# Accenture/AmpliGraph

Measured on AMD Instinct MI355X. Metric: training triples/sec (incl. negatives), ComplEx k=200 eta=20 FB15K-237-shaped, higher is better.
Workload: dtype f32; 1 GPU; synth-fb15k237 (uniform, seed 0) ComplEx k=200 eta=20 self_adversarial adam lr=1e-3, 10000 positives/GPU/step, tables resident in HBM, dense (non-lazy) Keras-legacy Adam every step; preset=C2, optimizer_mode=dense, deterministic=False, global_batch=10000, n_ents=14505, n_rels=237, row_floats=400, stored_row_floats=400, parallelism=single GPU

## Files before the change

### ampligraph_amd/csrc/kge_train_common.h

```cpp
#pragma once

#define KGE_FAST_ROTATE 1

#include "kge_device.h"
#include "kge_host.h"
#include "kge_loss.h"

static_assert(kge::ROTATE_FAST_FORMS, "kge_device.h was included before kge_train_common.h: this unit would train RotatE with the exact sqrt / division forms");

namespace kge {

struct __attribute__((aligned(16))) StageEntry {
    uint32_t pos;
    uint32_t meta;
    float g;
    uint32_t dest;
};

constexpr uint32_t ENTRY_LOCAL_MASK = 0x1FFFu;
__host__ __device__ __forceinline__ uint32_t entry_local(uint32_t meta) { return (meta >> 2) & ENTRY_LOCAL_MASK; }
constexpr int ENTRY_J_SHIFT = 16;

constexpr int LOSS_PARTS = 64;
constexpr int LOSS_PART_STRIDE = 16;

#ifndef KGE_TILE_RB
#define KGE_TILE_RB 8
#endif
constexpr uint32_t TILE_RB = KGE_TILE_RB;
__host__ __device__ __forceinline__ void tile_of_row(uint32_t row, uint32_t n_tiles, uint32_t rb, uint32_t& tile, uint32_t& local) {
    const uint32_t blk = row / rb;
    tile = blk % n_tiles;
    local = (blk / n_tiles) * rb + row % rb;
}
__host__ __device__ __forceinline__ int64_t row_of_tile(uint32_t tile, uint32_t local, uint32_t n_tiles, uint32_t rb) {
    return ((int64_t)(local / rb) * n_tiles + tile) * rb + local % rb;
}

constexpr int HOT_MAX = 64;
constexpr int HOT_REPL = 16;

struct TrainArgs {
    const float* ent;
    const float* rel;
    const float* rel_cs;
    const int32_t* triples;
    const int32_t* neg_override;
    float* g_ent;
    float* g_rel;
    double* loss_sum;
    double* loss_parts;
    float* pos_scores;
    float* neg_scores;
    int64_t B;
    int eta;
    int k;
    int K;
    int k_live;
    int nq;
    SampleCfg sc;
    ModelConst mc;
    amdkge_loss loss;
    float* stage_rows;
    int pos_atomic;
    int sign_off;
    int ns;
    int det;
    const uint8_t* hot_map;
    float* hot_buf;
    uint8_t* touched;
    uint32_t* sign_codes;
    StageEntry* st_lists;
    StageEntry* st_ovf;
    int* st_counters;
    int st_tile_rows, st_n_tiles, st_cap, st_ovf_cap, st_rb;
#ifdef KGE_ABLATE
    int dbg;
#endif
};

#ifdef KGE_ABLATE
#define KGE_DBG(a, bit) (((a).dbg & (bit)) != 0)
#else
#define KGE_DBG(a, bit) false
#endif

__device__ __forceinline__ void fold_loss_parts(double* parts, double* loss_sum, int lane, int lane_in_slot = 0) {
    static_assert(LOSS_PARTS == KGE_WAVE, "one partial per lane");
    const unsigned long long old = atomicExch(reinterpret_cast<unsigned long long*>(parts + (size_t)lane * LOSS_PART_STRIDE + lane_in_slot), 0ull);
    double t = __longlong_as_double((long long)old);
#pragma unroll
    for (int o = 32; o > 0; o >>= 1) t += __shfl_xor(t, o, 64);
    if (lane == 0 && loss_sum && t != 0.0) atomicAdd(loss_sum, t);
}

struct WaveWalk {
    float* sn;
    int lane;
    __device__ __forceinline__ int first() const { return lane; }
    __device__ __forceinline__ int stride() const { return KGE_WAVE; }
    __device__ __forceinline__ float load(int j) const { return sn[j]; }
    __device__ __forceinline__ void store(int j, float v) const { sn[j] = v; }
    __device__ __forceinline__ float sum(float v) const { return wave_sum(v); }
    __device__ __forceinline__ float max(float v) const { return wave_max(v); }
};

__device__ __forceinline__ bool entry_wanted(float coeff, float g) {
    return !(fabsf(g) < 1.17549435e-38f) || __float_as_uint(coeff) == 0x80000000u;
}


__device__ __forceinline__ void stage_draws(const TrainArgs& a, int64_t i, int ps, int first, int stride, int* sh_keep, int* sh_repl) {
    for (int j = first; j < a.eta; j += stride) {
        int keep, repl;
        if (a.neg_override) {
            const int64_t r = (int64_t)j * a.B + i;
            const int ns = a.neg_override[3 * r + 0], no = a.neg_override[3 * r + 2];
            keep = (ns == ps) ? 1 : 0;
            repl = keep ? no : ns;
        } else {
            draw_corruption(a.sc, i, j, keep, repl);
        }
        sh_keep[j] = keep;
        sh_repl[j] = repl;
    }
}

template <int MODEL>
__device__ __forceinline__ void stage_side_rows(const float (&s)[4][ModelTraits<MODEL>::NC], const float (&p)[4][ModelTraits<MODEL>::NC],
                                                const float (&o)[4][ModelTraits<MODEL>::NC], float* qa, float* qb, int k) {
    constexpr int NC = ModelTraits<MODEL>::NC;
    float va[NC][4], vb[NC][4];
#pragma unroll
    for (int u = 0; u < 4; ++u) {
        if constexpr (MODEL == AMDKGE_DISTMULT || MODEL == AMDKGE_COMPLEX) {
            float ds[NC], dp[NC], dd[NC];
            grad_unit<MODEL>(s[u], p[u], o[u], 1.f, ds, dp, dd);
#pragma unroll
            for (int h = 0; h < NC; ++h) { va[h][u] = dd[h]; vb[h][u] = ds[h]; }
        } else if constexpr (MODEL == AMDKGE_ROTATE) {
            const float cs = p[u][0], sn = p[u][1];
            va[0][u] = s[u][0] * cs - s[u][1] * sn; va[1][u] = s[u][0] * sn + s[u][1] * cs;
            vb[0][u] = o[u][0] * cs + o[u][1] * sn; vb[1][u] = o[u][1] * cs - o[u][0] * sn;
        } else {
#pragma unroll
            for (int h = 0; h < NC; ++h) { va[h][u] = s[u][h]; vb[h][u] = o[u][h]; }
        }
    }
#pragma unroll
    for (int h = 0; h < NC; ++h) {
        *reinterpret_cast<float4*>(qa + h * k) = make_float4(va[h][0], va[h][1], va[h][2], va[h][3]);
        *reinterpret_cast<float4*>(qb + h * k) = make_float4(vb[h][0], vb[h][1], vb[h][2], vb[h][3]);
    }
}

__device__ __forceinline__ void stage_append(const TrainArgs& a, int64_t i, uint32_t role, float g, uint32_t dest) {
    uint32_t tile, local;
    tile_of_row(dest, (uint32_t)a.st_n_tiles, (uint32_t)a.st_rb, tile, local);
    StageEntry* where;
    const int slotpos = atomicAdd(a.st_counters + (size_t)tile * 32, 1);
    if (slotpos < a.st_cap) {
        where = a.st_lists + (size_t)tile * a.st_cap + slotpos;
    } else {
        const int op = atomicAdd(a.st_counters + (size_t)a.st_n_tiles * 32, 1);
        if (op >= a.st_ovf_cap) return;
        where = a.st_ovf + op;
    }
    *where = StageEntry{(uint32_t)i, role | (local << 2), g, dest};
}

__host__ __device__ inline size_t sign_stash_bytes(int model, int eta, int CH) {
    return model == AMDKGE_TRANSE ? (size_t)256 * eta * CH : 0;
}

__host__ __device__ inline size_t slot_lds_bytes(int eta, int W) {
    const size_t b = (size_t)(eta + 1) * (3 + (W > 1 ? W : 2) + 1) * 4 + 8 + (W > 1 ? 64 * 4 : 0);
    return (b + 7) & ~(size_t)7;
}

template <int W>
__device__ __forceinline__ void slot_sync() {
    if constexpr (W == 1) {
        __builtin_amdgcn_fence(__ATOMIC_ACQ_REL, "wavefront");
        __builtin_amdgcn_wave_barrier();
    } else {
        __syncthreads();
    }
}

}
```

### ampligraph_amd/csrc/kge_train_kernel.h

```cpp
#pragma once
#include "kge_train_common.h"

namespace kge {

__device__ __forceinline__ void focus_apply(int nl, float x, float wgt, float& y, float& dfac) {
    float f, fp;
    switch (nl) {
        case AMDKGE_FOCUS_TANH: f = tanhf(x); fp = 1.f - f * f; break;
        case AMDKGE_FOCUS_SIGMOID: f = sigmoidf(x); fp = f * (1.f - f); break;
        case AMDKGE_FOCUS_SOFTPLUS: { const float e = 9999.f * expf(x); f = logf(1.f + e); fp = 1.f - 1.f / (1.f + e); } break;
        default: f = x; fp = 1.f; break;
    }
    y = f * wgt;
    dfac = fp * wgt;
}

struct OnePassState {
    float m;
    float S, Lw, Zs;
};

__device__ __forceinline__ float fast_exp(float x) {
    const float t = x * 1.4426950216293335f;
    const float r = fmaf(x, 1.4426950216293335f, -t) + x * 1.9259629911266175e-8f;
    const float v = __builtin_amdgcn_exp2f(t) * fmaf(r, 0.6931471805599453f, 1.f);
    return (x < -110.f) ? 0.f : v;
}
__device__ __forceinline__ void fast_sig_logsig(float y, float& sig, float& logsig_neg) {
    const float t = fast_exp(-fabsf(y));
    const float u = 1.f + t;
    const float r = __builtin_amdgcn_rcpf(u);
    sig = (y >= 0.f) ? r : t * r;
    logsig_neg = fminf(-y, 0.f) - (__builtin_amdgcn_logf(u) * 0.6931471805599453f + (t - (u - 1.f)) * r);
}

__device__ __forceinline__ float det_exp(float x) {
    x = (x != x) ? x : fminf(fmaxf(x, -80.f), 80.f);
    const float n = rintf(x * 1.4426950216293335f);
    const float r = (x - n * 0.693359375f) - n * -2.12194440e-4f;
    float p = 1.f / 5040.f;
    p = p * r + 1.f / 720.f;
    p = p * r + 1.f / 120.f;
    p = p * r + 1.f / 24.f;
    p = p * r + 1.f / 6.f;
    p = p * r + 0.5f;
    p = p * r + 1.f;
    p = p * r + 1.f;
    return ldexpf(p, (int)n);
}
__device__ __forceinline__ float det_log12(float u) {
    const float z = (u - 1.f) / (u + 1.f);
    const float w = z * z;
    float p = 1.f / 15.f;
    p = p * w + 1.f / 13.f;
    p = p * w + 1.f / 11.f;
    p = p * w + 1.f / 9.f;
    p = p * w + 1.f / 7.f;
    p = p * w + 1.f / 5.f;
    p = p * w + 1.f / 3.f;
    p = p * w + 1.f;
    return (2.f * z) * p;
}
__device__ __forceinline__ void det_sig_logsig(float y, float& sig, float& logsig_neg) {
    const float t = det_exp(-fabsf(y));
    const float u = 1.f + t;
    sig = (y >= 0.f) ? 1.f / u : t / u;
    logsig_neg = fminf(-y, 0.f) - (det_log12(u) + (t - (u - 1.f)) / u);
}
__device__ __forceinline__ void sig_logsig(bool det, float y, float& sig, float& logsig_neg) {
    if (det) det_sig_logsig(y, sig, logsig_neg); else fast_sig_logsig(y, sig, logsig_neg);
}
__device__ __forceinline__ float exp_any(bool det, float x) { return det ? det_exp(x) : fast_exp(x); }

__device__ __forceinline__ float onepass_coeff(const amdkge_loss& L, float P, float n, bool valid, OnePassState& st,
                                               float& c1, float& c2, bool det = false) {
    c1 = 0.f;
    c2 = 0.f;
    float rescale = 1.f;
    switch (L.kind) {
        case AMDKGE_LOSS_PAIRWISE: c1 = (valid && (L.margin - P + n >= 0.f)) ? 1.f : 0.f; break;
        case AMDKGE_LOSS_NLL: {
            const bool in = valid && in_clip(n);
            float sg, lsn;
            sig_logsig(det, clip_exp(n), sg, lsn);
            st.Lw += valid ? -lsn : 0.f;
            c1 = in ? sg : 0.f;
        } break;
        case AMDKGE_LOSS_ABSOLUTE_MARGIN: c1 = (valid && (L.margin + n >= 0.f)) ? 1.f : 0.f; break;
        case AMDKGE_LOSS_SELF_ADVERSARIAL: {
            const float x = L.alpha * n;
            const float gm = wave_max(valid ? x : -INFINITY);
            if (gm > st.m) {
                rescale = (st.m == -INFINITY) ? 0.f : exp_any(det, st.m - gm);
                st.S *= rescale; st.Lw *= rescale; st.m = gm;
            }
            const float u = valid ? exp_any(det, x - st.m) : 0.f;
            float sg, ell;
            sig_logsig(det, n + L.margin, sg, ell);
            st.S += u; st.Lw += valid ? u * ell : 0.f;
            c1 = valid ? u * (sg - L.alpha * ell) : 0.f;
            c2 = u;
        } break;
        default: {
            const bool in = valid && in_clip(n);
            const float ex = valid ? exp_any(det, clip_exp(n)) : 0.f;
            st.Zs += ex;
            c1 = in ? ex : 0.f;
        } break;
    }
    return rescale;
}

__device__ __forceinline__ void onepass_kappa(const amdkge_loss& L, float P, int eta, const OnePassState& st, float& k1, float& k2, bool det = false) {
    const float feta = (float)eta;
    const float red = loss_red(L, feta);
    k2 = 0.f;
    switch (L.kind) {
        case AMDKGE_LOSS_NLL: k1 = 1.f / loss_red(L, feta, 2.f); break;
        case AMDKGE_LOSS_SELF_ADVERSARIAL: k1 = 1.f / (st.S * red); k2 = L.alpha * (st.Lw / st.S) / (st.S * red); break;
        case AMDKGE_LOSS_MULTICLASS_NLL: {
            const float eP = exp_any(det, clip_exp(P));
            k1 = 1.f / ((st.Zs / red + eP) * red);
        } break;
        default: k1 = 1.f / red; break;
    }
}

__device__ __forceinline__ void onepass_finish(const amdkge_loss& L, float P, float* sn, int eta, int lane,
                                               const OnePassState& st, float& per, float& dP, bool det = false) {
    const float feta = (float)eta;
    float red = loss_red(L, feta);
    switch (L.kind) {
        case AMDKGE_LOSS_NLL: {
            red = loss_red(L, feta, 2.f);
            const bool inP = in_clip(P);
            float sgP, lsP;
            sig_logsig(det, -clip_exp(P), sgP, lsP);
            for (int j = lane; j < eta; j += KGE_WAVE) {
                const float n = sn[j];
                float sg, ls;
                sig_logsig(det, clip_exp(n), sg, ls);
                sn[j] = in_clip(n) ? sg / red : masked_zero(n);
            }
            per = (feta * -lsP + st.Lw) / red;
            dP = inP ? -feta * sgP / red : 0.f;
        } break;
        case AMDKGE_LOSS_SELF_ADVERSARIAL: {
            const float lbar = st.Lw / st.S;
            for (int j = lane; j < eta; j += KGE_WAVE) {
                const float n = sn[j];
                const float w = exp_any(det, L.alpha * n - st.m) / st.S;
                float sg, ell;
                sig_logsig(det, n + L.margin, sg, ell);
                sn[j] = computed_zero((w * sg - L.alpha * w * (ell - lbar)) / red, n);
            }
            float sgP, lsP;
            sig_logsig(det, -(L.margin + P), sgP, lsP);
            per = -lsP - lbar / red;
            dP = -sgP;
        } break;
        default: {
            const bool inP = in_clip(P);
            const float Pc = clip_exp(P);
            const float eP = exp_any(det, Pc);
            const float Z = st.Zs / red + eP;
            for (int j = lane; j < eta; j += KGE_WAVE) {
                const float n = sn[j];
                sn[j] = in_clip(n) ? exp_any(det, clip_exp(n)) / Z / red : masked_zero(n);
            }
            per = (det ? logf(Z) : __builtin_amdgcn_logf(Z) * 0.6931471805599453f) - Pc;
            dP = inP ? -1.f + eP / Z : 0.f;
        } break;
    }
}

template <int MODEL, int VEC, int W, int CH, bool STAGE = false, bool DET = false>
#ifdef KGE_F_WAVES
__attribute__((amdgpu_waves_per_eu(KGE_F_WAVES, KGE_F_WAVES)))
#else
__attribute__((amdgpu_waves_per_eu((DET && STAGE && MODEL == AMDKGE_COMPLEX && W == 1 && CH == 1) ? 3 : 1)))
#endif
__global__ __launch_bounds__(256) void train_fwdbwd_kernel(TrainArgs a) {
    using T = ModelTraits<MODEL>;
    constexpr int NC = T::NC;
    constexpr int SLOTS = 4 / W;
    constexpr int TS = KGE_WAVE * W;
    extern __shared__ __attribute__((aligned(16))) char smem[];

    const int tid = threadIdx.x;
    const int slot = tid / TS;
    const int ts = tid % TS;
    const int lane = tid & 63;
    const int wv = ts >> 6;
    const int eta = a.eta;
    const int64_t i_raw = (int64_t)blockIdx.x * SLOTS + slot;
    const bool active = i_raw < a.B;
    const int64_t i = active ? i_raw : (a.B - 1);

    const int e1 = eta + 1;
    const size_t per_slot = slot_lds_bytes(eta, W);
    char* base = smem + (size_t)slot * per_slot;
    float* sh_neg = reinterpret_cast<float*>(base);
    int* sh_repl = reinterpret_cast<int*>(base + (size_t)e1 * 4);
    int* sh_keep = reinterpret_cast<int*>(base + (size_t)e1 * 8);
    float* sh_part = reinterpret_cast<float*>(base + (((size_t)e1 * 12 + 7) & ~(size_t)7));
    float* sh_dfac = sh_part + (size_t)e1 * (W > 1 ? W : 2);
    const int focus_nl = a.loss.focus_nonlinearity;
    float focus_wp = 1.f, focus_wn = 1.f;
    if (focus_nl) {
        const float wi = a.loss.d_focus_w[i];
        focus_wp = a.loss.focus_beta + (1.f - a.loss.focus_beta) * (1.f - wi);
        focus_wn = a.loss.focus_beta + (1.f - a.loss.focus_beta) * wi;
    }
    float dPfac = 1.f;
    double* sh_loss = reinterpret_cast<double*>(smem + (size_t)SLOTS * per_slot);

    const int ps = a.triples[3 * i + 0], pp = a.triples[3 * i + 1], po = a.triples[3 * i + 2];

    stage_draws(a, i, ps, ts, TS, sh_keep, sh_repl);

    const float* rs = a.ent + (int64_t)ps * a.K;
    const bool rel_is_cs = (MODEL == AMDKGE_ROTATE) && a.rel_cs != nullptr;
    const float* rp = (rel_is_cs ? a.rel_cs : a.rel) + (int64_t)pp * a.K;
    const float* ro = a.ent + (int64_t)po * a.K;
    float s[CH][VEC][NC], p[CH][VEC][NC], o[CH][VEC][NC];
    bool qok[CH];
    int qoff[CH];
#pragma unroll
    for (int c = 0; c < CH; ++c) {
        const int q = ts + c * TS;
        qok[c] = q < a.nq;
        qoff[c] = (qok[c] ? q : 0) * VEC;
#pragma unroll
        for (int h = 0; h < NC; ++h) {
            const fvec<VEC> vs = ldg<VEC>(rs + qoff[c] + h * a.k);
            const fvec<VEC> vp = ldg<VEC>(rp + qoff[c] + h * a.k);
            const fvec<VEC> vo = ldg<VEC>(ro + qoff[c] + h * a.k);
#pragma unroll
            for (int u = 0; u < VEC; ++u) {
                s[c][u][h] = vs.v[u]; p[c][u][h] = vp.v[u]; o[c][u][h] = vo.v[u];
            }
        }
        if (!rel_is_cs) {
#pragma unroll
            for (int u = 0; u < VEC; ++u) prep_rel<MODEL>(a.mc, p[c][u]);
        }
    }
    float pad1[CH][VEC];
#pragma unroll
    for (int c = 0; c < CH; ++c)
#pragma unroll
        for (int u = 0; u < VEC; ++u) pad1[c][u] = (MODEL == AMDKGE_ROTATE && qoff[c] + u >= a.k_live) ? 1.f : 0.f;
    if constexpr (STAGE) {
        static_assert(!STAGE || VEC == 4, "staging uses the 16-byte layout");
        if (active && !KGE_DBG(a, 64)) {
            float* qa = a.stage_rows + ((int64_t)i * a.ns + 2) * a.K;
            float* qb = a.stage_rows + ((int64_t)i * a.ns + 3) * a.K;
#pragma unroll
            for (int c = 0; c < CH; ++c)
                if (qok[c]) stage_side_rows<MODEL>(s[c], p[c], o[c], qa + qoff[c], qb + qoff[c], a.k);
        }
    }
    slot_sync<W>();

    const float sgn_scale = a.mc.score_sign * a.mc.score_scale;

#ifndef KGE_PF
#define KGE_PF 6
#endif
    constexpr int PF = (CH * NC * VEC <= 8) ? (MODEL == AMDKGE_ROTATE && STAGE ? 3 : KGE_PF) : 2;
    auto load_row = [&](const float* re, float (&e)[CH][VEC][NC]) {
#pragma unroll
        for (int c = 0; c < CH; ++c)
#pragma unroll
            for (int h = 0; h < NC; ++h) {
                const fvec<VEC> ve = ldg<VEC>(re + qoff[c] + h * a.k);
#pragma unroll
                for (int u = 0; u < VEC; ++u) e[c][u][h] = ve.v[u];
            }
    };

    constexpr bool MULTI = W == 1 && (MODEL == AMDKGE_DISTMULT || MODEL == AMDKGE_TRANSE || (DET && MODEL == AMDKGE_COMPLEX));
    constexpr bool ONEPASS = STAGE && (MODEL == AMDKGE_DISTMULT || MODEL == AMDKGE_COMPLEX || MODEL == AMDKGE_ROTATE ||
                                       (MODEL == AMDKGE_TRANSE && W == 1 && CH == 1));
    constexpr bool SIGNSTASH = (MODEL == AMDKGE_TRANSE) && !ONEPASS && (STAGE || VEC == 4);
    unsigned char* sh_sign = reinterpret_cast<unsigned char*>(smem) + a.sign_off;
    float av1[2][CH][VEC][NC], av2[2][CH][VEC][NC];
    OnePassState ops{-INFINITY, 0.f, 0.f, 0.f};
    if constexpr (ONEPASS) {
        float qa[CH][VEC][NC], qb[CH][VEC][NC];
        float zmark[CH][VEC];
        uint32_t* const code_base = (MODEL == AMDKGE_TRANSE && a.sign_codes != nullptr)
                                        ? a.sign_codes + (int64_t)__builtin_amdgcn_readfirstlane((int)i) * eta * a.nq : nullptr;
        float part = 0.f;
#pragma unroll
        for (int c = 0; c < CH; ++c) {
            float acc = 0.f;
#pragma unroll
            for (int u = 0; u < VEC; ++u) {
                float ds[NC], dp[NC], dd[NC];
                if constexpr (MODEL == AMDKGE_TRANSE) {
                    ds[0] = 0.f; dd[0] = s[c][u][0] + p[c][u][0];
                    zmark[c][u] = (qok[c] && qoff[c] + u < a.k_live) ? 0.f : __builtin_nanf("");
                } else if constexpr (MODEL == AMDKGE_ROTATE) {
                    ds[0] = 0.f; ds[1] = 0.f;
                    dd[0] = s[c][u][0] * p[c][u][0] - s[c][u][1] * p[c][u][1];
                    dd[1] = s[c][u][0] * p[c][u][1] + s[c][u][1] * p[c][u][0];
                } else {
                    grad_unit<MODEL>(s[c][u], p[c][u], o[c][u], 1.f, ds, dp, dd);
                }
#pragma unroll
                for (int h = 0; h < NC; ++h) {
                    qa[c][u][h] = dd[h]; qb[c][u][h] = ds[h];
                    av1[0][c][u][h] = 0.f; av1[1][c][u][h] = 0.f; av2[0][c][u][h] = 0.f; av2[1][c][u][h] = 0.f;
                }
                acc += score_unit<MODEL, DET>(s[c][u], p[c][u], o[c][u]);
            }
            part += qok[c] ? acc : 0.f;
        }
        float* sh_red = sh_dfac + e1;
        int grp_no = 0;
        float P1;
        if constexpr (W == 1) {
            P1 = sgn_scale * wave_sum(part);
        } else {
            const float w0 = wave_sum(part);
            if (lane == 0) sh_red[2 * W * PF + wv] = w0;
            __syncthreads();
            float t0 = 0.f;
#pragma unroll
            for (int w = 0; w < W; ++w) t0 += sh_red[2 * W * PF + w];
            P1 = sgn_scale * t0;
        }
        if (focus_nl) focus_apply(focus_nl, P1, focus_wp, P1, dPfac);
        if (lane == 0) sh_neg[eta] = P1;
        int* sh_perm = reinterpret_cast<int*>(sh_part);
        int nkeep = 0;
        for (int jb = 0; jb < eta; jb += KGE_WAVE) {
            const int j = jb + lane;
            nkeep += __popcll(__ballot(j < eta && sh_keep[j] != 0));
        }
        {
            int offk = 0, offn = nkeep;
            for (int jb = 0; jb < eta; jb += KGE_WAVE) {
                const int j = jb + lane;
                const bool valid = j < eta;
                const bool k = valid && sh_keep[j] != 0;
                const unsigned long long mk = __ballot(k), mn = __ballot(valid && !k);
                const unsigned long long mine = k ? mk : mn;
                const int before = __builtin_amdgcn_mbcnt_hi((unsigned)(mine >> 32), __builtin_amdgcn_mbcnt_lo((unsigned)mine, 0));
                if (valid) {
                    const int pos = (k ? offk : offn) + before;
                    if constexpr (MULTI) *reinterpret_cast<int2*>(sh_perm + 2 * pos) = make_int2(j, sh_repl[j]);
                    else sh_perm[pos] = j;
                }
                offk += __popcll(mk); offn += __popcll(mn);
            }
        }
        slot_sync<W>();
        [[maybe_unused]] const WaveMultiSel msel = wave_multi_sel(lane);
        [[maybe_unused]] const int mslot = lane < 8 ? wave_multi_slot(lane) : 8;
#pragma unroll
        for (int d = 0; d < 2; ++d) {
            const int p_begin = d == 0 ? 0 : nkeep, p_end = d == 0 ? nkeep : eta;
            for (int p0 = p_begin; p0 < p_end; p0 += PF) {
                float e[PF][CH][VEC][NC];
                int jv[PF];
                float nv = 0.f;
                int jl = 0;
                if constexpr (MULTI) {
                    const int2 pe = *reinterpret_cast<const int2*>(sh_perm + 2 * min(p0 + min(mslot, PF - 1), p_end - 1));
                    jl = pe.x;
#pragma unroll
                    for (int f = 0; f < PF; ++f) {
                        jv[f] = __builtin_amdgcn_readlane(pe.x, wave_multi_lane(f));
                        load_row(a.ent + (int64_t)(KGE_DBG(a, 8) ? ps : __builtin_amdgcn_readlane(pe.y, wave_multi_lane(f))) * a.K, e[f]);
                    }
                } else {
#pragma unroll
                    for (int f = 0; f < PF; ++f) {
                        jv[f] = __builtin_amdgcn_readfirstlane(sh_perm[min(p0 + f, p_end - 1)]);
                        load_row(a.ent + (int64_t)(KGE_DBG(a, 8) ? ps : __builtin_amdgcn_readfirstlane(sh_repl[jv[f]])) * a.K, e[f]);
                    }
                }
                [[maybe_unused]] float accv[PF];
                unsigned long long zero_m = 0ull;
#pragma unroll
                for (int f = 0; f < PF; ++f) {
                    float acc = 0.f;
#pragma unroll
                    for (int c = 0; c < CH; ++c) {
                        float t = 0.f;
                        if constexpr (MODEL == AMDKGE_TRANSE) {
#pragma unroll
                            for (int u = 0; u < VEC; ++u) {
                                const float dj = (d == 0) ? (qa[c][u][0] - e[f][c][u][0]) : ((e[f][c][u][0] + p[c][u][0]) - o[c][u][0]);
                                e[f][c][u][0] = dj;
                                t += fabsf(dj);
                                zero_m |= __ballot(dj == zmark[c][u]);
                            }
                            if (a.sign_codes && active && p0 + f < p_end && qok[c]) {
                                const unsigned t01 = __builtin_amdgcn_perm(__float_as_uint(e[f][c][1][0]), __float_as_uint(e[f][c][0][0]), 0x0c0c0703u);
                                const unsigned t23 = __builtin_amdgcn_perm(__float_as_uint(e[f][c][3][0]), __float_as_uint(e[f][c][2][0]), 0x07030c0cu);
                                uint32_t* crow = code_base + (uint32_t)(jv[f] * a.nq);
                                crow[qoff[c] >> 2] = t01 | t23;
                            }
                        } else if constexpr (MODEL == AMDKGE_ROTATE) {
#pragma unroll
                            for (int u = 0; u < VEC; ++u) {
                                float zr, zi;
                                if (d == 0) {
                                    zr = qa[c][u][0] - e[f][c][u][0]; zi = qa[c][u][1] - e[f][c][u][1];
                                } else {
                                    zr = e[f][c][u][0] * p[c][u][0] - e[f][c][u][1] * p[c][u][1] - o[c][u][0];
                                    zi = e[f][c][u][0] * p[c][u][1] + e[f][c][u][1] * p[c][u][0] - o[c][u][1];
                                }
                                const float m = kge_sqrt_t<DET>(zr * zr + zi * zi);
                                t += m;
                                const float inv = kge_div_t<DET>(1.f, m + pad1[c][u]);
                                e[f][c][u][0] = zr * inv; e[f][c][u][1] = zi * inv;
                            }
                        } else {
#pragma unroll
                            for (int u = 0; u < VEC; ++u)
#pragma unroll
                                for (int h = 0; h < NC; ++h) t = fmaf(d == 0 ? qa[c][u][h] : qb[c][u][h], e[f][c][u][h], t);
                        }
                        if constexpr (MULTI && CH == 1) acc = qok[c] ? t : 0.f; else acc += qok[c] ? t : 0.f;
                    }
                    if constexpr (MULTI) {
                        accv[f] = acc;
                    } else if constexpr (W == 1) {
                        const float n = sgn_scale * wave_sum(acc);
                        nv = (lane == f) ? n : nv;
                        jl = (lane == f) ? jv[f] : jl;
                    } else {
                        const float w1 = wave_sum(acc);
                        if (lane == 0) sh_red[((grp_no & 1) * W + wv) * PF + f] = w1;
                        jl = (lane == f) ? jv[f] : jl;
                    }
                }
                if constexpr (MULTI) {
                    nv = sgn_scale * wave_sum_multi<PF>(accv, msel);
                }
                if constexpr (MODEL == AMDKGE_TRANSE) zero_m |= __ballot(nv != nv);
                if constexpr (W > 1) {
                    __syncthreads();
                    if (lane < PF) {
                        float t1 = 0.f;
#pragma unroll
                        for (int w = 0; w < W; ++w) t1 += sh_red[((grp_no & 1) * W + w) * PF + lane];
                        nv = sgn_scale * t1;
                    }
                    ++grp_no;
                }
                const bool lane_valid = (MULTI ? mslot : lane) < min(PF, p_end - p0);
                float dfl = 1.f;
                if (focus_nl) focus_apply(focus_nl, nv, focus_wn, nv, dfl);
                if (lane_valid) {
                    sh_neg[jl] = nv;
                    if (focus_nl) sh_dfac[jl] = dfl;
                }
                float c1l, c2l;
                const float rs = onepass_coeff(a.loss, P1, nv, lane_valid, ops, c1l, c2l, DET);
                c1l *= dfl; c2l *= dfl;
                if (rs != 1.f) {
#pragma unroll
                    for (int dd = 0; dd < 2; ++dd)
#pragma unroll
                        for (int c = 0; c < CH; ++c)
#pragma unroll
                            for (int u = 0; u < VEC; ++u)
#pragma unroll
                                for (int h = 0; h < NC; ++h) { av1[dd][c][u][h] *= rs; av2[dd][c][u][h] *= rs; }
                }
                const bool two = a.loss.kind == AMDKGE_LOSS_SELF_ADVERSARIAL;
#pragma unroll
                for (int f = 0; f < PF; ++f) {
                    const int fl = MULTI ? wave_multi_lane(f) : f;
                    const float c1 = __int_as_float(__builtin_amdgcn_readlane(__float_as_int(c1l), fl));
                    const float c2 = __int_as_float(__builtin_amdgcn_readlane(__float_as_int(c2l), fl));
                    if constexpr (MODEL == AMDKGE_TRANSE) {
                        if (zero_m == 0ull) {
#pragma unroll
                            for (int c = 0; c < CH; ++c)
#pragma unroll
                                for (int u = 0; u < VEC; ++u) {
                                    const unsigned db = __float_as_uint(e[f][c][u][0]);
                                    av1[d][c][u][0] += __uint_as_float(__builtin_amdgcn_bitop3_b32(db, 0x80000000u, __float_as_uint(c1), 0x6a));
                                    if (two) av2[d][c][u][0] += __uint_as_float(__builtin_amdgcn_bitop3_b32(db, 0x80000000u, __float_as_uint(c2), 0x6a));
                                }
                        } else {
#pragma unroll
                            for (int c = 0; c < CH; ++c)
#pragma unroll
                                for (int u = 0; u < VEC; ++u) {
                                    const float dj = e[f][c][u][0];
                                    const float sg = (dj > 0.f) ? 1.f : ((dj < 0.f) ? -1.f : dj);
                                    av1[d][c][u][0] += c1 * sg;
                                    if (two) av2[d][c][u][0] += c2 * sg;
                                }
                        }
                        continue;
                    }
#pragma unroll
                    for (int c = 0; c < CH; ++c)
#pragma unroll
                        for (int u = 0; u < VEC; ++u)
#pragma unroll
                            for (int h = 0; h < NC; ++h) av1[d][c][u][h] = fmaf(c1, e[f][c][u][h], av1[d][c][u][h]);
                    if (two) {
#pragma unroll
                        for (int c = 0; c < CH; ++c)
#pragma unroll
                            for (int u = 0; u < VEC; ++u)
#pragma unroll
                                for (int h = 0; h < NC; ++h) av2[d][c][u][h] = fmaf(c2, e[f][c][u][h], av2[d][c][u][h]);
                    }
                }
            }
        }
        ops.S = wave_sum(ops.S); ops.Lw = wave_sum(ops.Lw); ops.Zs = wave_sum(ops.Zs);
#pragma unroll
        for (int c = 0; c < CH; ++c) {
#pragma unroll
            for (int h = 0; h < NC; ++h) {
                const fvec<VEC> vs = ldg<VEC>(rs + qoff[c] + h * a.k);
                const fvec<VEC> vp = ldg<VEC>(rp + qoff[c] + h * a.k);
                const fvec<VEC> vo = ldg<VEC>(ro + qoff[c] + h * a.k);
#pragma unroll
                for (int u = 0; u < VEC; ++u) { s[c][u][h] = vs.v[u]; p[c][u][h] = vp.v[u]; o[c][u][h] = vo.v[u]; }
            }
            if (!rel_is_cs) {
#pragma unroll
                for (int u = 0; u < VEC; ++u) prep_rel<MODEL>(a.mc, p[c][u]);
            }
        }
    }
    for (int j0 = -1; j0 < (ONEPASS ? -1 : eta); j0 += PF) {
        float e[PF][CH][VEC][NC];
        int keepv[PF];
#pragma unroll
        for (int f = 0; f < PF; ++f) {
            const int j = min(j0 + f, eta - 1);
            keepv[f] = (j < 0) ? 1 : __builtin_amdgcn_readfirstlane(sh_keep[j]);
            const int64_t er = (j < 0) ? (int64_t)po : (int64_t)__builtin_amdgcn_readfirstlane(sh_repl[j]);
            load_row(a.ent + er * a.K, e[f]);
        }
#pragma unroll
        for (int f = 0; f < PF; ++f) {
            const int j = j0 + f;
            if (j >= eta) break;
            float part = 0.f;
#pragma unroll
            for (int c = 0; c < CH; ++c) {
                float acc = 0.f;
                if constexpr (SIGNSTASH) {
                    unsigned code = 0;
                    float dv[VEC];
#pragma unroll
                    for (int u = 0; u < VEC; ++u) {
                        const float d = keepv[f] ? (s[c][u][0] + p[c][u][0] - e[f][c][u][0]) : (e[f][c][u][0] + p[c][u][0] - o[c][u][0]);
                        dv[u] = d;
                        acc += fabsf(d);
                        code |= ((d > 0.f) ? 1u : ((d < 0.f) ? 2u : ((d == d) ? 0u : 3u))) << (2 * u);
                    }
                    if (j >= 0) sh_sign[((size_t)j * CH + c) * 256 + tid] = (unsigned char)code;
                    if constexpr (STAGE && VEC == 4) {
                        if (a.sign_codes && active && j >= 0 && qok[c])
                            a.sign_codes[((int64_t)i * eta + j) * a.nq + (qoff[c] >> 2)] =
                                __builtin_amdgcn_perm(__float_as_uint(dv[1]), __float_as_uint(dv[0]), 0x0c0c0703u) |
                                __builtin_amdgcn_perm(__float_as_uint(dv[3]), __float_as_uint(dv[2]), 0x07030c0cu);
                    }
                } else {
#pragma unroll
                    for (int u = 0; u < VEC; ++u)
                        acc += keepv[f] ? score_unit<MODEL, DET>(s[c][u], p[c][u], e[f][c][u]) : score_unit<MODEL, DET>(e[f][c][u], p[c][u], o[c][u]);
                }
                part += qok[c] ? acc : 0.f;
            }
            const float tot = wave_sum(part);
            const int jj = (j < 0) ? eta : j;
            if constexpr (W > 1) {
                if (lane == 0) sh_part[wv * e1 + jj] = tot;
            } else {
                if (lane == 0) sh_neg[jj] = sgn_scale * tot;
            }
        }
    }
    if constexpr (W > 1 && !ONEPASS) {
        __syncthreads();
        for (int j = ts; j < e1; j += TS) {
            float t2 = 0.f;
#pragma unroll
            for (int w = 0; w < W; ++w) t2 += sh_part[w * e1 + j];
            sh_neg[j] = sgn_scale * t2;
        }
    }
    slot_sync<W>();
    if constexpr (!ONEPASS) {
        if (focus_nl) {
            for (int j = ts; j < eta; j += TS) {
                float y, dfc;
                focus_apply(focus_nl, sh_neg[j], focus_wn, y, dfc);
                sh_neg[j] = y; sh_dfac[j] = dfc;
            }
            float y;
            focus_apply(focus_nl, sh_neg[eta], focus_wp, y, dPfac);
            slot_sync<W>();
            if (ts == 0) sh_neg[eta] = y;
            slot_sync<W>();
        }
    }
    const float P = sh_neg[eta];

    if (active && a.neg_scores)
        for (int j = ts; j < eta; j += TS) a.neg_scores[(int64_t)j * a.B + i] = sh_neg[j];
    if (active && a.pos_scores && ts == 0) a.pos_scores[i] = P;
    if constexpr (W > 1) __syncthreads();

    float per = 0.f, dP = 0.f;
    if constexpr (ONEPASS) {
        if (a.loss.kind == AMDKGE_LOSS_PAIRWISE || a.loss.kind == AMDKGE_LOSS_ABSOLUTE_MARGIN) { if (W == 1 || wv == 0) loss_call(a.loss, P, eta, WaveWalk{sh_neg, lane}, per, dP); }
        else if (W == 1 || wv == 0) onepass_finish(a.loss, P, sh_neg, eta, lane, ops, per, dP, DET);
    } else if (W == 1 || wv == 0) loss_call(a.loss, P, eta, WaveWalk{sh_neg, lane}, per, dP);
    if constexpr (W > 1) {
        if (wv == 0 && lane == 0) sh_part[0] = dP;
        __syncthreads();
        dP = sh_part[0];
    } else {
        slot_sync<W>();
    }
    if (focus_nl) {
        dP *= dPfac;
        for (int j = ts; j < eta; j += TS) sh_neg[j] *= sh_dfac[j];
        slot_sync<W>();
    }
    if (ts == 0) sh_loss[slot] = active ? (double)per : 0.0;
    if constexpr (STAGE) {
        if (active && !KGE_DBG(a, 32))
            for (int j = ts; j < eta + (a.pos_atomic ? 0 : 2); j += TS) {
                uint32_t dest, role;
                float g, coeff = 1.f;
                if (j < eta) {
                    dest = (uint32_t)sh_repl[j]; role = sh_keep[j] ? 0u : 1u; coeff = sh_neg[j]; g = coeff * sgn_scale;
                    if (a.sign_codes) role |= (uint32_t)j << ENTRY_J_SHIFT;
                }
                else { dest = (uint32_t)(j == eta ? ps : po); role = (j == eta) ? 2u : 3u; g = 1.f; }
                if (!entry_wanted(coeff, g)) continue;
                if (j >= eta && a.hot_map && a.hot_map[dest]) continue;
                stage_append(a, i, role, g, dest);
            }
    }

    float gs[CH][VEC][NC], gp[CH][VEC][NC], go[CH][VEC][NC];
#pragma unroll
    for (int c = 0; c < CH; ++c)
#pragma unroll
        for (int u = 0; u < VEC; ++u) {
            float ds[NC], dp[NC], dd[NC];
            grad_unit<MODEL, DET>(s[c][u], p[c][u], o[c][u], dP * sgn_scale, ds, dp, dd, pad1[c][u]);
#pragma unroll
            for (int h = 0; h < NC; ++h) { gs[c][u][h] = ds[h]; gp[c][u][h] = dp[h]; go[c][u][h] = dd[h]; }
        }

    float* stage = reinterpret_cast<float*>(smem + (size_t)SLOTS * per_slot + SLOTS * sizeof(double)) + (size_t)(tid >> 6) * a.K;
    auto emit_row = [&](float* grow, const float (&gr)[CH][VEC][NC], int nfloats, float mul) {
        if constexpr (VEC == 1) {
#pragma unroll
            for (int c = 0; c < CH; ++c)
#pragma unroll
                for (int h = 0; h < NC; ++h)
                    if (qok[c] && qoff[c] + h * a.k < nfloats) atomic_add_f32(grow + qoff[c] + h * a.k, gr[c][0][h] * mul);
        } else if constexpr (W == 1) {
#pragma unroll
            for (int c = 0; c < CH; ++c)
#pragma unroll
                for (int h = 0; h < NC; ++h)
                    if (qok[c])
                        *reinterpret_cast<float4*>(stage + qoff[c] + h * a.k) =
                            make_float4(gr[c][0][h] * mul, gr[c][1][h] * mul, gr[c][2][h] * mul, gr[c][3][h] * mul);
            __builtin_amdgcn_fence(__ATOMIC_ACQ_REL, "wavefront");
            __builtin_amdgcn_wave_barrier();
            for (int idx = lane; idx < nfloats; idx += KGE_WAVE) atomic_add_f32(grow + idx, stage[idx]);
            __builtin_amdgcn_fence(__ATOMIC_ACQ_REL, "wavefront");
            __builtin_amdgcn_wave_barrier();
        } else {
            static_assert(VEC == 1 || W == 1 || W == 4, "multi-wave LDS-transposed emit needs one slot per workgroup");
            float* srow = reinterpret_cast<float*>(smem + (size_t)SLOTS * per_slot + SLOTS * sizeof(double));
#pragma unroll
            for (int c = 0; c < CH; ++c)
#pragma unroll
                for (int h = 0; h < NC; ++h)
                    if (qok[c])
                        *reinterpret_cast<float4*>(srow + qoff[c] + h * a.k) =
                            make_float4(gr[c][0][h] * mul, gr[c][1][h] * mul, gr[c][2][h] * mul, gr[c][3][h] * mul);
            __syncthreads();
            for (int idx = ts; idx < nfloats; idx += TS) atomic_add_f32(grow + idx, srow[idx]);
            __syncthreads();
        }
    };

    if constexpr (ONEPASS) {
        float k1, k2;
        onepass_kappa(a.loss, P, eta, ops, k1, k2, DET);
        k1 *= sgn_scale; k2 *= sgn_scale;
        float k1s[2] = {k1, k1}, k2s[2] = {k2, k2};
        if (k1 != k1 || k2 != k2) {
#pragma unroll
            for (int d = 0; d < 2; ++d) {
                bool any = false;
                for (int j = lane; j < eta; j += KGE_WAVE) {
                    const float cj = sh_neg[j];
                    any |= ((sh_keep[j] != 0) == (d == 0)) && !(cj == 0.f);
                }
                if (__ballot(any) == 0ull) { k1s[d] = 0.f; k2s[d] = 0.f; }
            }
        }
#pragma unroll
        for (int c = 0; c < CH; ++c)
#pragma unroll
            for (int u = 0; u < VEC; ++u) {
                float eo[NC], es[NC], ds[NC], dp[NC], dd[NC];
#pragma unroll
                for (int h = 0; h < NC; ++h) {
                    eo[h] = k1s[0] * av1[0][c][u][h] + k2s[0] * av2[0][c][u][h];
                    es[h] = k1s[1] * av1[1][c][u][h] + k2s[1] * av2[1][c][u][h];
                }
                if constexpr (MODEL == AMDKGE_TRANSE) {
                    const bool lv = qoff[c] + u < a.k_live;
                    const float Go = lv ? eo[0] : 0.f, Gs = lv ? es[0] : 0.f;
                    gs[c][u][0] += Go; gp[c][u][0] += Go + Gs; go[c][u][0] -= Gs;
                    continue;
                }
                if constexpr (MODEL == AMDKGE_ROTATE) {
                    const float cs = p[c][u][0], sn = p[c][u][1];
                    const float Ar = s[c][u][0] * cs - s[c][u][1] * sn, Ai = s[c][u][0] * sn + s[c][u][1] * cs;
                    gs[c][u][0] += eo[0] * cs + eo[1] * sn;
                    gs[c][u][1] += eo[1] * cs - eo[0] * sn;
                    go[c][u][0] -= es[0]; go[c][u][1] -= es[1];
                    gp[c][u][0] += (eo[1] * Ar - eo[0] * Ai) + (es[1] * o[c][u][0] - es[0] * o[c][u][1]);
                    continue;
                }
                grad_unit<MODEL>(s[c][u], p[c][u], eo, 1.f, ds, dp, dd);
#pragma unroll
                for (int h = 0; h < NC; ++h) { gs[c][u][h] += ds[h]; gp[c][u][h] += dp[h]; }
                grad_unit<MODEL>(es, p[c][u], o[c][u], 1.f, ds, dp, dd);
#pragma unroll
                for (int h = 0; h < NC; ++h) { go[c][u][h] += dd[h]; gp[c][u][h] += dp[h]; }
            }
    }
    const bool do_neg_atomics = active && !KGE_DBG(a, 1);
    if constexpr (SIGNSTASH) {
        for (int j = 0; j < eta; ++j) {
            const int keep = __builtin_amdgcn_readfirstlane(sh_keep[j]);
            const float g = __int_as_float(__builtin_amdgcn_readfirstlane(__float_as_int(sh_neg[j]))) * sgn_scale;
            float gr[CH][VEC][NC];
#pragma unroll
            for (int c = 0; c < CH; ++c) {
                const unsigned code = sh_sign[((size_t)j * CH + c) * 256 + tid];
#pragma unroll
                for (int u = 0; u < VEC; ++u) {
                    const unsigned b = (code >> (2 * u)) & 3u;
                    const float sg = (b == 1u) ? g : ((b == 2u) ? -g : ((b == 3u) ? __builtin_nanf("") : 0.f));
                    if (keep) { gs[c][u][0] += sg; gp[c][u][0] += sg; gr[c][u][0] = -sg; }
                    else { go[c][u][0] += -sg; gp[c][u][0] += sg; gr[c][u][0] = sg; }
                }
            }
            if constexpr (!STAGE) {
                if (do_neg_atomics) emit_row(a.g_ent + (int64_t)__builtin_amdgcn_readfirstlane(sh_repl[j]) * a.K, gr, a.K, 1.f);
            }
        }
    }
    for (int j0 = 0; j0 < ((ONEPASS || SIGNSTASH || KGE_DBG(a, 4)) ? 0 : eta); j0 += PF) {
        float e[PF][CH][VEC][NC];
        int keepv[PF];
        int64_t erv[PF];
        float gv[PF];
#pragma unroll
        for (int f = 0; f < PF; ++f) {
            const int j = min(j0 + f, eta - 1);
            keepv[f] = __builtin_amdgcn_readfirstlane(sh_keep[j]);
            erv[f] = (int64_t)__builtin_amdgcn_readfirstlane(sh_repl[j]);
            gv[f] = __int_as_float(__builtin_amdgcn_readfirstlane(__float_as_int(sh_neg[j]))) * sgn_scale;
            load_row(a.ent + erv[f] * a.K, e[f]);
        }
#pragma unroll
        for (int f = 0; f < PF; ++f) {
            if (j0 + f >= eta) break;
            const float g = gv[f];
            float gr[CH][VEC][NC];
#pragma unroll
            for (int c = 0; c < CH; ++c) {
#pragma unroll
                for (int u = 0; u < VEC; ++u) {
                    float ds[NC], dp[NC], dd[NC];
                    if (keepv[f]) {
                        grad_unit<MODEL, DET>(s[c][u], p[c][u], e[f][c][u], g, ds, dp, dd, pad1[c][u]);
#pragma unroll
                        for (int h = 0; h < NC; ++h) { gs[c][u][h] += ds[h]; gp[c][u][h] += dp[h]; gr[c][u][h] = dd[h]; }
                    } else {
                        grad_unit<MODEL, DET>(e[f][c][u], p[c][u], o[c][u], g, ds, dp, dd, pad1[c][u]);
#pragma unroll
                        for (int h = 0; h < NC; ++h) { go[c][u][h] += dd[h]; gp[c][u][h] += dp[h]; gr[c][u][h] = ds[h]; }
                    }
                }
            }
            if constexpr (!STAGE) { if (do_neg_atomics) emit_row(a.g_ent + erv[f] * a.K, gr, a.K, 1.f); }
        }
    }

    __syncthreads();
    if (tid == 0 && !KGE_DBG(a, 128)) {
        double t = 0.0;
#pragma unroll
        for (int q = 0; q < SLOTS; ++q) t += sh_loss[q];
        atomicAdd(a.loss_parts + (size_t)(blockIdx.x & (LOSS_PARTS - 1)) * LOSS_PART_STRIDE, t);
    }

    if constexpr (STAGE) {
        if (active && !KGE_DBG(a, 64)) {
            if (a.pos_atomic) {
                emit_row(a.g_ent + (int64_t)ps * a.K, gs, a.K, 1.f);
                emit_row(a.g_ent + (int64_t)po * a.K, go, a.K, 1.f);
                if (a.touched && ts == 0) { a.touched[ps] = 1; a.touched[po] = 1; }
            } else {
                if (a.hot_map) {
                    const int hs = a.hot_map[ps], ho = a.hot_map[po];
                    if (hs) emit_row(a.hot_buf + ((int64_t)(hs - 1) * HOT_REPL + (blockIdx.x & (HOT_REPL - 1))) * a.K, gs, a.K, 1.f);
                    if (ho) emit_row(a.hot_buf + ((int64_t)(ho - 1) * HOT_REPL + (blockIdx.x & (HOT_REPL - 1))) * a.K, go, a.K, 1.f);
                }
                float* ps_ = a.stage_rows + ((int64_t)i * a.ns + 0) * a.K;
                float* po_ = a.stage_rows + ((int64_t)i * a.ns + 1) * a.K;
#pragma unroll
                for (int c = 0; c < CH; ++c) {
                    if (!qok[c]) continue;
#pragma unroll
                    for (int h = 0; h < NC; ++h) {
                        *reinterpret_cast<float4*>(ps_ + qoff[c] + h * a.k) = make_float4(gs[c][0][h], gs[c][1][h], gs[c][2][h], gs[c][3][h]);
                        *reinterpret_cast<float4*>(po_ + qoff[c] + h * a.k) = make_float4(go[c][0][h], go[c][1][h], go[c][2][h], go[c][3][h]);
                    }
                }
            }
        }
        if (active && a.det) {
            const float mul = (MODEL == AMDKGE_ROTATE) ? 1.f / a.mc.phase_div : 1.f;
            float* pr_ = a.stage_rows + ((int64_t)i * a.ns + 4) * a.K;
#pragma unroll
            for (int c = 0; c < CH; ++c) {
                if (!qok[c]) continue;
#pragma unroll
                for (int h = 0; h < NC; ++h)
                    *reinterpret_cast<float4*>(pr_ + qoff[c] + h * a.k) = make_float4(gp[c][0][h] * mul, gp[c][1][h] * mul, gp[c][2][h] * mul, gp[c][3][h] * mul);
            }
        } else if (active && !KGE_DBG(a, 2)) {
            if constexpr (MODEL == AMDKGE_ROTATE) emit_row(a.g_rel + (int64_t)pp * a.K, gp, a.k, 1.f / a.mc.phase_div);
            else emit_row(a.g_rel + (int64_t)pp * a.K, gp, a.K, 1.f);
        }
    } else if (active && !KGE_DBG(a, 2)) {
        emit_row(a.g_ent + (int64_t)ps * a.K, gs, a.K, 1.f);
        emit_row(a.g_ent + (int64_t)po * a.K, go, a.K, 1.f);
        if constexpr (MODEL == AMDKGE_ROTATE) {
            emit_row(a.g_rel + (int64_t)pp * a.K, gp, a.k, 1.f / a.mc.phase_div);
        } else {
            emit_row(a.g_rel + (int64_t)pp * a.K, gp, a.K, 1.f);
        }
    }
}

}
```

### ampligraph_amd/csrc/kge_train_stage.hip

```cpp
#include "kge_train_kernel.h"
#include "kge_train_tiled.h"

namespace kge {

template <int MODEL, int W, int CHF, bool DET>
static int launch_forward_v(TrainArgs& f, hipStream_t st) {
    constexpr int slots = 4 / W;
    size_t shmem = (size_t)slots * slot_lds_bytes(f.eta, W) + slots * sizeof(double) + (W == 1 ? 4 : 1) * (size_t)f.K * 4;
    f.sign_off = (int)shmem;
    if (W != 1 || CHF != 1) shmem += sign_stash_bytes(MODEL, f.eta, CHF);
    if (shmem > 64 * 1024) {
        static PerDeviceOnce attr;
        if (int rc = ensure_dynamic_lds(attr, {(const void*)train_fwdbwd_kernel<MODEL, 4, W, CHF, true, DET>}, 160 * 1024, "train_forward_stage")) return rc;
    }
    const unsigned grid = KGE_DBG(f, 8192) ? 0u : (unsigned)((f.B + slots - 1) / slots);
    if (grid) hipLaunchKernelGGL((train_fwdbwd_kernel<MODEL, 4, W, CHF, true, DET>), dim3(grid), dim3(256), shmem, st, f);
    return check_launch("train_forward_stage");
}
template <int MODEL, int W, int CHF>
static int launch_forward(TrainArgs& f, hipStream_t st) {
    return f.det ? launch_forward_v<MODEL, W, CHF, true>(f, st) : launch_forward_v<MODEL, W, CHF, false>(f, st);
}

template <int MODEL>
static int forward_by_width(TrainArgs& f, hipStream_t st) {
    if (f.nq <= 64) return launch_forward<MODEL, 1, 1>(f, st);
    if (f.nq <= 128) return launch_forward<MODEL, 1, 2>(f, st);
    if (f.nq <= 256) return launch_forward<MODEL, 4, 1>(f, st);
    return launch_forward<MODEL, 4, 2>(f, st);
}

int run_forward_stage(int model, TrainArgs& f, hipStream_t st) {
#define KGE_RUN(MODEL) return forward_by_width<MODEL>(f, st)
    KGE_MODEL_DISPATCH(model, KGE_RUN)
#undef KGE_RUN
}

}
```

Baseline: 1.540 billion triples/s.

## Launch forward-stage kernel with one wave per block and per-wave loss atomics

For the non-deterministic W==1 staging path, the forward/backward kernel now derives its slot count from blockDim, and the launcher defaults to 64-thread blocks holding one triple each instead of 256-thread blocks holding four. The end-of-block __syncthreads and shared-memory loss reduction are replaced by each wave atomically adding its loss to the partial buffer. This removes block-level barriers and lets slow slots stop holding their block mates back. In exchange it launches four times as many blocks and puts more double atomics on the loss partials. An env var selects the old block modes.

```diff
diff --git a/ampligraph_amd/csrc/kge_train_common.h b/ampligraph_amd/csrc/kge_train_common.h
--- a/ampligraph_amd/csrc/kge_train_common.h
+++ b/ampligraph_amd/csrc/kge_train_common.h
@@ -66,6 +66,7 @@
     int sign_off;
     int ns;
     int det;
+    int wave_loss;
     const uint8_t* hot_map;
     float* hot_buf;
     uint8_t* touched;
diff --git a/ampligraph_amd/csrc/kge_train_kernel.h b/ampligraph_amd/csrc/kge_train_kernel.h
--- a/ampligraph_amd/csrc/kge_train_kernel.h
+++ b/ampligraph_amd/csrc/kge_train_kernel.h
@@ -183,8 +183,9 @@
 __global__ __launch_bounds__(256) void train_fwdbwd_kernel(TrainArgs a) {
     using T = ModelTraits<MODEL>;
     constexpr int NC = T::NC;
-    constexpr int SLOTS = 4 / W;
     constexpr int TS = KGE_WAVE * W;
+    constexpr bool UNIT_BY_LAUNCH = STAGE && !DET && W == 1;
+    const int SLOTS = UNIT_BY_LAUNCH ? (int)blockDim.x / TS : 4 / W;
     extern __shared__ __attribute__((aligned(16))) char smem[];
 
     const int tid = threadIdx.x;
@@ -636,7 +637,11 @@
         for (int j = ts; j < eta; j += TS) sh_neg[j] *= sh_dfac[j];
         slot_sync<W>();
     }
-    if (ts == 0) sh_loss[slot] = active ? (double)per : 0.0;
+    const bool wave_loss = UNIT_BY_LAUNCH && a.wave_loss;
+    if (ts == 0) {
+        if (!wave_loss) sh_loss[slot] = active ? (double)per : 0.0;
+        else if (active && !KGE_DBG(a, 128)) atomicAdd(a.loss_parts + (size_t)(blockIdx.x & (LOSS_PARTS - 1)) * LOSS_PART_STRIDE, (double)per);
+    }
     if constexpr (STAGE) {
         if (active && !KGE_DBG(a, 32))
             for (int j = ts; j < eta + (a.pos_atomic ? 0 : 2); j += TS) {
@@ -810,12 +815,13 @@
         }
     }
 
-    __syncthreads();
-    if (tid == 0 && !KGE_DBG(a, 128)) {
-        double t = 0.0;
-#pragma unroll
-        for (int q = 0; q < SLOTS; ++q) t += sh_loss[q];
-        atomicAdd(a.loss_parts + (size_t)(blockIdx.x & (LOSS_PARTS - 1)) * LOSS_PART_STRIDE, t);
+    if (!wave_loss) {
+        __syncthreads();
+        if (tid == 0 && !KGE_DBG(a, 128)) {
+            double t = 0.0;
+            for (int q = 0; q < SLOTS; ++q) t += sh_loss[q];
+            atomicAdd(a.loss_parts + (size_t)(blockIdx.x & (LOSS_PARTS - 1)) * LOSS_PART_STRIDE, t);
+        }
     }
 
     if constexpr (STAGE) {
diff --git a/ampligraph_amd/csrc/kge_train_stage.hip b/ampligraph_amd/csrc/kge_train_stage.hip
--- a/ampligraph_amd/csrc/kge_train_stage.hip
+++ b/ampligraph_amd/csrc/kge_train_stage.hip
@@ -1,12 +1,30 @@
+#include <cstdlib>
+#include <cstring>
+
 #include "kge_train_kernel.h"
 #include "kge_train_tiled.h"
 
 namespace kge {
 
+enum class ForwardUnit { WAVE, BLOCK, BLOCK_NOBARRIER };
+constexpr ForwardUnit FORWARD_UNIT_DEFAULT = ForwardUnit::WAVE;
+static ForwardUnit forward_unit() {
+    const char* e = getenv("AMDKGE_F_UNIT");
+    if (!e) return FORWARD_UNIT_DEFAULT;
+    if (!strcmp(e, "wave")) return ForwardUnit::WAVE;
+    if (!strcmp(e, "block")) return ForwardUnit::BLOCK;
+    if (!strcmp(e, "block_nobarrier")) return ForwardUnit::BLOCK_NOBARRIER;
+    return FORWARD_UNIT_DEFAULT;
+}
+
 template <int MODEL, int W, int CHF, bool DET>
 static int launch_forward_v(TrainArgs& f, hipStream_t st) {
-    constexpr int slots = 4 / W;
-    size_t shmem = (size_t)slots * slot_lds_bytes(f.eta, W) + slots * sizeof(double) + (W == 1 ? 4 : 1) * (size_t)f.K * 4;
+    ForwardUnit unit = (W == 1 && !DET) ? forward_unit() : ForwardUnit::BLOCK;
+    if (MODEL == AMDKGE_TRANSE && CHF != 1 && unit == ForwardUnit::WAVE) unit = ForwardUnit::BLOCK_NOBARRIER;
+    const int slots = unit == ForwardUnit::WAVE ? 1 : 4 / W;
+    const int threads = slots * W * 64;
+    f.wave_loss = unit != ForwardUnit::BLOCK;
+    size_t shmem = (size_t)slots * slot_lds_bytes(f.eta, W) + slots * sizeof(double) + (W == 1 ? slots : 1) * (size_t)f.K * 4;
     f.sign_off = (int)shmem;
     if (W != 1 || CHF != 1) shmem += sign_stash_bytes(MODEL, f.eta, CHF);
     if (shmem > 64 * 1024) {
@@ -14,7 +32,7 @@
         if (int rc = ensure_dynamic_lds(attr, {(const void*)train_fwdbwd_kernel<MODEL, 4, W, CHF, true, DET>}, 160 * 1024, "train_forward_stage")) return rc;
     }
     const unsigned grid = KGE_DBG(f, 8192) ? 0u : (unsigned)((f.B + slots - 1) / slots);
-    if (grid) hipLaunchKernelGGL((train_fwdbwd_kernel<MODEL, 4, W, CHF, true, DET>), dim3(grid), dim3(256), shmem, st, f);
+    if (grid) hipLaunchKernelGGL((train_fwdbwd_kernel<MODEL, 4, W, CHF, true, DET>), dim3(grid), dim3(threads), shmem, st, f);
     return check_launch("train_forward_stage");
 }
 template <int MODEL, int W, int CHF>
```

Result: no change. 1.552 billion triples/s, median of 6 (+0.7%).
